# 0xPARC/plonkathon

Measured on NVIDIA H100. Metric: plonk_proofs_per_s_2^20_gates, higher is better.
Workload: dtype u256 (BN254 Fr/Fq integers, 8x32-bit Montgomery limbs)

## Files before the change

plonkathon_b200/csrc/prover.cu:

```cuda
#include <algorithm>
#include <cerrno>
#include <sys/random.h>

#include "common.cuh"
#include "comm.cuh"
#include "transcript.cuh"
#include "prover.cuh"
#include "memory_plan.cuh"

namespace pb200 {

void ntt_run(Context* ctx, const Fr* in, Fr* out, int log_n, bool inverse, uint64_t n_in, const Fr* in_scale,
             const Fr* out_scale);
void ntt_run_on(Context* ctx, cudaStream_t stream, Fr* tmp, const Fr* in, Fr* out, int log_n, bool inverse,
                uint64_t n_in, const Fr* in_scale, const Fr* out_scale, uint64_t in_mul, uint64_t in_add);
void ntt_run_fold(Context* ctx, cudaStream_t stream, Fr* tmp, const Fr* in, Fr* out, int log_n, bool inverse,
                  uint64_t n_in, const Fr* in_scale, const Fr* out_scale, uint64_t in_mul, uint64_t in_add, uint32_t fold);
void ntt_sharded(Context* ctx, const Fr* const* in, Fr* const* out, int count, int log_n, bool inverse);
void ntt_shard_local(Context* ctx, const Fr* const* in, int count, int log_n, bool inverse, uint64_t in_mul,
                     uint64_t in_add, int log_g, int rank, Comm* cm);
void ntt_shard_combine(Context* ctx, const Fr* sub, uint64_t rank_stride, Fr* out, int log_n, bool inverse,
                       uint64_t limit, const Fr* post_scale, uint32_t* nonzero, int log_g, int rank);
uint32_t msm_default_window(uint64_t n, bool fixed_base);

static void coset_extend(Prover* P, cudaStream_t stream, Fr* tmp, const Fr* coeff, Fr* out, const Fr* shift_pow) {
  ntt_run_fold(P->ctx, stream, tmp, coeff, out, P->log_ext, false, P->n, shift_pow, nullptr, 1, 0, P->fold);
}

static void interpolate(Prover* P, const Fr* const* lag, Fr* const* coeff, int count) {
  if (P->world > 1) {
    ntt_sharded(P->ctx, lag, coeff, count, P->log_n, true);
  } else {
    for (int k = 0; k < count; k++) ntt_run(P->ctx, lag[k], coeff[k], P->log_n, true, P->n, nullptr, nullptr);
  }
}

static void launch_coset_ext_async(Prover* P, int first, int count, int done_event) {
  Context* ctx = P->ctx;
  if (!ctx->aux_stream) {
    PB_CUDA(cudaStreamCreateWithFlags(&ctx->aux_stream, cudaStreamNonBlocking));
    for (auto& e : ctx->aux_ev) PB_CUDA(cudaEventCreateWithFlags(&e, cudaEventDisableTiming));
  }
  P->aux_tmp.ensure(P->n_ext * 32);
  PB_CUDA(cudaEventRecord(ctx->aux_ev[3], ctx->stream));
  PB_CUDA(cudaStreamWaitEvent(ctx->aux_stream, ctx->aux_ev[3], 0));
  for (int k = first; k < first + count; k++) {
    coset_extend(P, ctx->aux_stream, P->aux_tmp.as<Fr>(), P->coeff[k].as<Fr>(), P->ext[k].as<Fr>(), P->gpow.as<Fr>());
    if (k == 3 && P->zw_separate)
      coset_extend(P, ctx->aux_stream, P->aux_tmp.as<Fr>(), P->coeff[3].as<Fr>(), P->ext[5].as<Fr>(), P->gpow_w.as<Fr>());
  }
  PB_CUDA(cudaEventRecord(ctx->aux_ev[done_event], ctx->aux_stream));
}
void launch_powers(Context* ctx, Fr* out, uint64_t n, const Fr& base, const Fr& scale);
Fr fr_from_u64(uint64_t x);
Fr fr_root_of_unity(int log_n);
void fr_to_mont(Context* ctx, const Fr* in, Fr* out, uint64_t n);
struct Srs;
void srs_msm(Context* ctx, Srs* srs, const Fr* d_scalars, uint64_t m, bool scalars_mont, uint8_t* out_xy, int* is_identity);
uint64_t srs_size(Srs* s);

#define PB_GRID(n, t) (unsigned)(((n) + (t)-1) / (t)), (t)

__device__ __forceinline__ Fr ldg_fr(const Fr* p) {
  const uint4* q = reinterpret_cast<const uint4*>(p);
  uint4 a = __ldg(q), b = __ldg(q + 1);
  Fr r;
  r.v[0] = a.x; r.v[1] = a.y; r.v[2] = a.z; r.v[3] = a.w;
  r.v[4] = b.x; r.v[5] = b.y; r.v[6] = b.z; r.v[7] = b.w;
  return r;
}

static Fr load_fr_checked(const uint8_t* h) {
  Fr a;
  memcpy(a.v, h, 32);
  PB_CHECK(fp_is_canonical(a), "public input not reduced below the field modulus");
  return a;
}

// ... 198 lines not shown
  if (j < n4) den[j] = fp_mul(n_mont, fp_sub(ldg_fr(X + j), wi));
}

struct QuotientArgs {
  const Fr *A, *B, *C, *Z, *Zw, *PI;
  const Fr *QL, *QR, *QM, *QO, *QC, *S1, *S2, *S3;
  const Fr *L0, *X;
  Fr zh_inv[4];
  Fr alpha, alpha2, beta, gamma, one;
  uint64_t n4;
  uint64_t zw_shift;
  uint32_t world, rank;
  int pi_cnt;
  const Fr* pi_basis[8];
  Fr pi_coef[8];
  CustomTerms custom;
};
struct ZkCoset { Fr w[4][12]; };
struct ZkNextCoset { Fr w[4][24]; };
template <bool ZK_NEXT> struct ZkCosetOf { using type = ZkCoset; };
template <> struct ZkCosetOf<true> { using type = ZkNextCoset; };
static_assert(sizeof(QuotientArgs) + sizeof(Fr*) + sizeof(ZkNextCoset) <= 4096,
              "k_quotient's parameters must fit the 4 KiB parameter space");
template <bool ZK, bool NEXT>
__global__ void __launch_bounds__(128) k_quotient(QuotientArgs q, Fr* T, typename ZkCosetOf<ZK && NEXT>::type zk) {
  uint64_t j = (uint64_t)blockIdx.x * blockDim.x + threadIdx.x;
  if (j >= q.n4) return;
  uint64_t jw = j + q.zw_shift >= q.n4 ? j + q.zw_shift - q.n4 : j + q.zw_shift;
  Fr a = ldg_fr(q.A + j), b = ldg_fr(q.B + j), c = ldg_fr(q.C + j);
  auto quad = [&](Fr y, int i) {
    if constexpr (ZK && NEXT) {
      const uint32_t k = (uint32_t)j & 3;
      const Fr x = ldg_fr(q.X + j);
      y = fp_add(y, fp_add(fp_mul(fp_add(fp_mul(zk.w[k][i], x), zk.w[k][i + 1]), x), zk.w[k][i + 2]));
    }
    return y;
  };
  if constexpr (ZK && NEXT) {
    a = quad(a, 0);
    b = quad(b, 3);
    c = quad(c, 6);
  } else if constexpr (ZK) {
    const uint32_t k = (uint32_t)(j * q.world + q.rank) & 3;
    const Fr x = ldg_fr(q.X + j);
    a = fp_add(a, fp_add(fp_mul(zk.w[k][0], x), zk.w[k][1]));
    b = fp_add(b, fp_add(fp_mul(zk.w[k][2], x), zk.w[k][3]));
    c = fp_add(c, fp_add(fp_mul(zk.w[k][4], x), zk.w[k][5]));
  }
  Fr gate = fp_mul(a, ldg_fr(q.QL + j));
  gate = fp_add(gate, fp_mul(b, ldg_fr(q.QR + j)));
  gate = fp_add(gate, fp_mul(fp_mul(a, b), ldg_fr(q.QM + j)));
  gate = fp_add(gate, fp_mul(c, ldg_fr(q.QO + j)));
  Fr pi = Fr::zero();
  if (q.pi_cnt > 0) {
    for (int i = 0; i < q.pi_cnt; i++) pi = fp_add(pi, fp_mul(q.pi_coef[i], ldg_fr(q.pi_basis[i] + j)));
  } else if (q.PI) {
    pi = ldg_fr(q.PI + j);
  }
  gate = fp_add(gate, fp_add(pi, ldg_fr(q.QC + j)));
  if constexpr (NEXT) {
    const Fr an = quad(ldg_fr(q.A + jw), 15), bn = quad(ldg_fr(q.B + jw), 18), cn = quad(ldg_fr(q.C + jw), 21);
    gate = custom_gate_sum_next(q.custom, j, a, b, c, an, bn, cn, gate);
  } else {
    gate = custom_gate_sum(q.custom, j, a, b, c, gate);
  }
  Fr ag = fp_add(a, q.gamma), bg = fp_add(b, q.gamma), cg = fp_add(c, q.gamma);
  Fr bx = fp_mul(q.beta, ldg_fr(q.X + j));
  Fr bx2 = fp_dbl(bx), bx3 = fp_add(bx2, bx);
  Fr z = ldg_fr(q.Z + j), zw = ldg_fr(q.Zw + jw);
  if constexpr (ZK && NEXT) {
    z = quad(z, 9);
    zw = quad(zw, 12);
  } else if constexpr (ZK) {
    const uint32_t k = (uint32_t)(j * q.world + q.rank) & 3;
    const Fr x = ldg_fr(q.X + j);
    z = fp_add(z, fp_add(fp_mul(fp_add(fp_mul(zk.w[k][6], x), zk.w[k][7]), x), zk.w[k][8]));
    zw = fp_add(zw, fp_add(fp_mul(fp_add(fp_mul(zk.w[k][9], x), zk.w[k][10]), x), zk.w[k][11]));
  }
  Fr p1 = fp_mul(fp_mul(fp_mul(fp_add(ag, bx), fp_add(bg, bx2)), fp_add(cg, bx3)), z);
  Fr p2 = fp_mul(fp_mul(fp_mul(fp_add(ag, fp_mul(q.beta, ldg_fr(q.S1 + j))), fp_add(bg, fp_mul(q.beta, ldg_fr(q.S2 + j)))),
                        fp_add(cg, fp_mul(q.beta, ldg_fr(q.S3 + j)))),
                 zw);
  Fr perm = fp_mul(q.alpha, fp_sub(p1, p2));
  Fr l0 = fp_mul(q.alpha2, fp_mul(fp_sub(z, q.one), ldg_fr(q.L0 + j)));
  Fr num = fp_add(fp_add(gate, perm), l0);
  T[j] = fp_mul(num, q.zh_inv[(j * q.world + q.rank) & 3]);
}

__global__ void k_count_nonzero(const Fr* v, uint64_t n, uint32_t* cnt) {
  uint64_t i = (uint64_t)blockIdx.x * blockDim.x + threadIdx.x;
  if (i < n && !ldg_fr(v + i).is_zero()) atomicAdd(cnt, 1u);
}

struct EvalArgs { const Fr* poly[8]; Fr x_nc[8]; uint64_t n; uint32_t NC; };
__global__ void __launch_bounds__(128) k_horner_strided(EvalArgs a, Fr* H) {
  uint32_t c = blockIdx.x * blockDim.x + threadIdx.x;
  uint32_t p = blockIdx.y;
  if (c >= a.NC) return;
  const Fr* co = a.poly[p];
  uint64_t steps = a.n / a.NC;
  Fr acc = Fr::zero();
  for (uint64_t k = steps; k-- > 0;) acc = fp_add(fp_mul(acc, a.x_nc[p]), ldg_fr(co + k * a.NC + c));
  H[(uint64_t)p * a.NC + c] = acc;
}

struct LinCombArgs { const Fr* vec[26]; Fr w[26]; Fr c0; int count; uint64_t n, first; };
static_assert(5 + PB_MAX_CUSTOM + 10 + 7 <= 26, "round 5's largest batch must fit LinCombArgs");
static_assert(5 + PB_MAX_CUSTOM + 10 + 3 <= 26, "round 5's batch with a shuffle must fit LinCombArgs");
static_assert(7 + 1 <= 26, "round 5's zero-knowledge tail with a shuffle must fit LinCombArgs");
// ... 95 lines not shown

struct LookupChallenges { Fr delta, eps, one_d, eps_one_d; };
__global__ void k_lookup_z2_terms(const Fr* t, const Fr* f, const Fr* h1, const Fr* h2, LookupChallenges ch, uint64_t n,
                                  Fr* num, Fr* den) {
  uint64_t i = (uint64_t)blockIdx.x * blockDim.x + threadIdx.x;
  if (i >= n) return;
  const uint64_t i1 = i + 1 == n ? 0 : i + 1;
  const Fr x1 = ldg_fr(h1 + i), x2 = ldg_fr(h2 + i);
  num[i] = fp_mul(fp_mul(ch.one_d, fp_add(ch.eps, ldg_fr(f + i))),
                  fp_add(fp_add(ch.eps_one_d, ldg_fr(t + i)), fp_mul(ch.delta, ldg_fr(t + i1))));
  den[i] = fp_mul(fp_add(fp_add(ch.eps_one_d, x1), fp_mul(ch.delta, x2)),
                  fp_add(fp_add(ch.eps_one_d, x2), fp_mul(ch.delta, ldg_fr(h1 + i1))));
}

struct LookupQuotientArgs {
  const Fr *A, *B, *C, *QK, *QT, *T, *F, *H1, *H2, *Z2, *L0;
  Fr zh_inv[4];
  Fr eta, eta2, eta3, delta, eps, one_d, eps_one_d, alpha3, alpha4, alpha5, one;
  uint64_t n4;
};
struct ZkLookupCoset { const Fr* X; Fr w[4][18]; };
static_assert(sizeof(LookupQuotientArgs) + sizeof(Fr*) + sizeof(ZkLookupCoset) <= 4096,
              "k_quotient_lookup's parameters must fit the 4 KiB parameter space");
template <bool ZK>
__global__ void __launch_bounds__(128) k_quotient_lookup(LookupQuotientArgs q, Fr* out, ZkLookupCoset zk) {
  uint64_t j = (uint64_t)blockIdx.x * blockDim.x + threadIdx.x;
  if (j >= q.n4) return;
  const uint64_t jw = j + 4 >= q.n4 ? j + 4 - q.n4 : j + 4;
  const uint32_t k = (uint32_t)j & 3;
  const Fr x = ZK ? ldg_fr(zk.X + j) : Fr::zero();
  auto lin = [&](Fr y, int i) {
    if constexpr (ZK) y = fp_add(y, fp_add(fp_mul(zk.w[k][i], x), zk.w[k][i + 1]));
    return y;
  };
  auto quad = [&](Fr y, int i) {
    if constexpr (ZK) y = fp_add(y, fp_add(fp_mul(fp_add(fp_mul(zk.w[k][i], x), zk.w[k][i + 1]), x), zk.w[k][i + 2]));
    return y;
  };
  const Fr f = lin(ldg_fr(q.F + j), 2);
  Fr w = lin(fp_add(ldg_fr(q.A + j), fp_add(fp_mul(q.eta, ldg_fr(q.B + j)), fp_mul(q.eta2, ldg_fr(q.C + j)))), 0);
  Fr acc = fp_mul(ldg_fr(q.QK + j), fp_sub(w, f));
  if (q.QT) acc = fp_add(acc, fp_mul(q.eta3, ldg_fr(q.QT + j)));
  acc = fp_mul(q.alpha3, acc);
  const Fr z2 = quad(ldg_fr(q.Z2 + j), 12), h1 = quad(ldg_fr(q.H1 + j), 4), h2 = lin(ldg_fr(q.H2 + j), 10);
  Fr p1 = fp_mul(fp_mul(fp_mul(z2, q.one_d), fp_add(q.eps, f)),
                 fp_add(fp_add(q.eps_one_d, ldg_fr(q.T + j)), fp_mul(q.delta, ldg_fr(q.T + jw))));
  Fr p2 = fp_mul(fp_mul(quad(ldg_fr(q.Z2 + jw), 15), fp_add(fp_add(q.eps_one_d, h1), fp_mul(q.delta, h2))),
                 fp_add(fp_add(q.eps_one_d, h2), fp_mul(q.delta, quad(ldg_fr(q.H1 + jw), 7))));
  acc = fp_add(acc, fp_mul(q.alpha4, fp_sub(p1, p2)));
  acc = fp_add(acc, fp_mul(q.alpha5, fp_mul(fp_sub(z2, q.one), ldg_fr(q.L0 + j))));
  out[j] = fp_add(out[j], fp_mul(acc, q.zh_inv[j & 3]));
}

struct ShuffleChallenges { Fr theta, theta2, kappa; };
__global__ void k_shuffle_terms(const Fr* A, const Fr* B, const Fr* C, const Fr* QIN, const Fr* QOUT,
                                ShuffleChallenges ch, uint64_t n, Fr* num, Fr* den) {
  uint64_t i = (uint64_t)blockIdx.x * blockDim.x + threadIdx.x;
  if (i >= n) return;
  const Fr t = fp_add(ch.kappa, fp_add(ldg_fr(A + i), fp_add(fp_mul(ch.theta, ldg_fr(B + i)),
                                                              fp_mul(ch.theta2, ldg_fr(C + i)))));
  num[i] = ldg_fr(QIN + i).is_zero() ? Fr::one() : t;
  den[i] = ldg_fr(QOUT + i).is_zero() ? Fr::one() : t;
}

struct ShuffleQuotientArgs {
  const Fr *A, *B, *C, *QIN, *QOUT, *Z3, *L0;
  Fr zh_inv[4];
  Fr theta, theta2, kappa_m1, alpha3, alpha4, one;
  uint64_t n4;
};
struct ZkShuffleCoset { const Fr* X; Fr w[4][9]; };
static_assert(sizeof(ShuffleQuotientArgs) + sizeof(Fr*) + sizeof(ZkShuffleCoset) <= 4096,
              "k_quotient_shuffle's parameters must fit the 4 KiB parameter space");
template <bool ZK>
__global__ void __launch_bounds__(128) k_quotient_shuffle(ShuffleQuotientArgs q, Fr* out, ZkShuffleCoset zk) {
  uint64_t j = (uint64_t)blockIdx.x * blockDim.x + threadIdx.x;
  if (j >= q.n4) return;
  const uint64_t jw = j + 4 >= q.n4 ? j + 4 - q.n4 : j + 4;
  const uint32_t kz = (uint32_t)j & 3;
  const Fr x = ZK ? ldg_fr(zk.X + j) : Fr::zero();
  auto quad = [&](Fr y, int i) {
    if constexpr (ZK) y = fp_add(y, fp_add(fp_mul(fp_add(fp_mul(zk.w[kz][i], x), zk.w[kz][i + 1]), x), zk.w[kz][i + 2]));
    return y;
  };
  const Fr k = fp_add(q.kappa_m1, quad(fp_add(ldg_fr(q.A + j), fp_add(fp_mul(q.theta, ldg_fr(q.B + j)),
                                                                        fp_mul(q.theta2, ldg_fr(q.C + j)))), 0));
  const Fr z3 = quad(ldg_fr(q.Z3 + j), 3);
  Fr acc = fp_sub(fp_mul(quad(ldg_fr(q.Z3 + jw), 6), fp_add(q.one, fp_mul(ldg_fr(q.QOUT + j), k))),
                  fp_mul(z3, fp_add(q.one, fp_mul(ldg_fr(q.QIN + j), k))));
  acc = fp_add(fp_mul(q.alpha3, acc), fp_mul(q.alpha4, fp_mul(fp_sub(z3, q.one), ldg_fr(q.L0 + j))));
  out[j] = fp_add(out[j], fp_mul(acc, q.zh_inv[j & 3]));
}


static void upload_mont(Context* ctx, DevBuf& dst, const uint8_t* h, uint64_t n) {
  dst.ensure(n * 32);
  PB_CUDA(cudaMemcpyAsync(dst.p, h, n * 32, cudaMemcpyHostToDevice, ctx->stream));
  fr_to_mont(ctx, dst.as<Fr>(), dst.as<Fr>(), n);
}

Comm* ctx_comm(Context* ctx);

static void ensure_pi_basis(Prover* P, int count) {
  Context* ctx = P->ctx;
  const uint64_t n = P->n, ne = P->n_ext;
  cudaStream_t st = ctx->stream;
  if ((int)P->pi_basis.size() >= count) return;
  Fr w = fr_root_of_unity(P->log_n);
  DevBuf den(ne * 32);
  for (int i = (int)P->pi_basis.size(); i < count; i++) {
    Fr wi = fp_pow_u64(w, (uint64_t)i);
    Four zh;
    for (int k = 0; k < 4; k++) zh.v[k] = fp_mul(wi, P->zh[k]);
    P->pi_basis.emplace_back(ne * 32);
// ... 120 lines not shown
  for (int k = 0; k < Prover::CUSTOM0 + n_custom; k++) {
    upload_mont(ctx, P->sel_lag[k], k < Prover::CUSTOM0 ? h_pk[k] : h_custom[k - Prover::CUSTOM0], n);
    P->sel_coeff[k].alloc(n * 32);
    ntt_run(ctx, P->sel_lag[k].as<Fr>(), P->sel_coeff[k].as<Fr>(), log_n, true, n, nullptr, nullptr);
    P->sel_ext[k].alloc(ne * 32);
    if (!P->sliced)
      coset_extend(P.get(), st, nullptr, P->sel_coeff[k].as<Fr>(), P->sel_ext[k].as<Fr>(), P->gpow.as<Fr>());
  }
  for (int k = 0; k < 4; k++) P->lag[k].alloc(n * 32);
  for (int k = 0; k < 5; k++) { P->coeff[k].alloc(n * 32); P->ext[k].alloc(ne * 32); }
  if (P->zw_separate) P->ext[5].alloc(ne * 32);
  P->pi_lag.alloc(n * 32);
  if (P->world > 1) {
    P->tq.alloc(3 * n * 32);
    P->tq_loc.alloc(ne * 32);
  } else if (P->sliced) {
    P->tq.alloc(3 * n * 32);
  } else {
    P->tq.alloc(n4 * 32);
  }
  for (int k = 0; k < 5; k++) P->tmp[k].alloc(n * 32);
  P->flags.alloc(64);
  if (const char* e = getenv("PB200_OVERLAP")) P->overlap = atoi(e) != 0;
  if (P->sliced) P->overlap = false;
  PB_CUDA(cudaStreamSynchronize(st));
  PB_CUDA(cudaGetLastError());
  return P.release();
}

void prover_destroy(Prover* p) { delete p; }

static uint32_t read_flag(Prover* P, int idx) {
  uint32_t v;
  PB_CUDA(cudaMemcpyAsync(&v, P->flags.as<uint32_t>() + idx, 4, cudaMemcpyDeviceToHost, P->ctx->stream));
  PB_CUDA(cudaStreamSynchronize(P->ctx->stream));
  return v;
}

Comm* ctx_comm(Context* ctx);

static void eval_polys(Prover* P, int count, const Fr* const* polys, const Fr* xs, Fr* out) {
  Context* ctx = P->ctx;
  const uint64_t n = P->n / (uint64_t)P->world, lo = n * (uint64_t)P->rank;
  uint32_t NC1 = (uint32_t)std::min<uint64_t>(n, 4096);
  uint32_t NC2 = std::min<uint32_t>(NC1, 32);
  ctx->scratch[0].ensure((size_t)count * (NC1 + NC2) * 32);
// ... 604 lines not shown
    slice_lagrange(P, r, 0, Fr::one(), P->pi_basis[0].as<Fr>());
    if (P->pi_sparse) {
      bool first = true;
      for (uint64_t i = 0; i < P->n_public; i++) {
        if (P->pub_neg[i].is_zero()) continue;
        slice_lagrange(P, r, i, P->pub_neg[i], first ? P->ext[4].as<Fr>() : P->tmp[1].as<Fr>());
        if (!first) fr_vec_op(ctx, 0, P->ext[4].as<Fr>(), P->tmp[1].as<Fr>(), Fr::zero(), P->ext[4].as<Fr>(), n, 0);
        first = false;
      }
      if (first && P->n_public) PB_CUDA(cudaMemsetAsync(P->ext[4].p, 0, n * 32, st));
    }
    q.rank = (uint32_t)r;
    Fr* slot = ctx->gather.as<Fr>() + (uint64_t)r * n;
    k_quotient<false, false><<<PB_GRID(n, 128), 0, st>>>(q, slot, zk);
    ctx->launches++;
    const Fr* te = slot;
    ntt_shard_local(ctx, &te, 1, P->log_n + 2, true, 1, 0, 2, r, nullptr);
  }
  PB_CUDA(cudaMemsetAsync(P->flags.p, 0, 64, st));
  ntt_shard_combine(ctx, ctx->gather.as<Fr>(), n, P->tq.as<Fr>(), P->log_n + 2, true, 3 * n, P->ginv_pow.as<Fr>(),
                    P->flags.as<uint32_t>(), 2, 0);
}

void prover_round3(Prover* P, const Fr& alpha_c, const Fr& cofactor_c) {
  Context* ctx = P->ctx;
  const uint64_t n = P->n, n4 = 4 * n, ne = P->n_ext;
  cudaStream_t st = ctx->stream;
  P->alpha = fp_to_mont(alpha_c);
  P->fft_cofactor = fp_to_mont(cofactor_c);
  if (P->sliced) {
    quotient_sliced(P);
    PB_CHECK(read_flag(P, 0) == 0, "AssertionError: quotient has degree >= 3n (prover.py:205-208)");
    const Fr* t123[3] = {P->tq.as<Fr>(), P->tq.as<Fr>() + n, P->tq.as<Fr>() + 2 * n};
    P->commit_batch(t123, 3, n, P->fields[F_T_LO]);
    return;
  }
  if (P->overlap) {
    PB_CUDA(cudaStreamWaitEvent(st, ctx->aux_ev[0], 0));
    PB_CUDA(cudaStreamWaitEvent(st, ctx->aux_ev[1], 0));
  }
  for (int k = (P->overlap ? 4 : 0); k < (P->pi_sparse ? 4 : 5); k++) {
    coset_extend(P, st, nullptr, P->coeff[k].as<Fr>(), P->ext[k].as<Fr>(), P->gpow.as<Fr>());
    if (k == 3 && P->zw_separate)
      coset_extend(P, st, nullptr, P->coeff[3].as<Fr>(), P->ext[5].as<Fr>(), P->gpow_w.as<Fr>());
  }
  QuotientArgs q;
  q.pi_cnt = P->pi_sparse ? (int)P->n_public : 0;
  for (int i = 0; i < q.pi_cnt; i++) { q.pi_basis[i] = P->pi_basis[i].as<Fr>(); q.pi_coef[i] = P->pub_neg[i]; }
  q.A = P->ext[0].as<Fr>(); q.B = P->ext[1].as<Fr>(); q.C = P->ext[2].as<Fr>(); q.Z = P->ext[3].as<Fr>();
  q.Zw = P->zw_separate ? P->ext[5].as<Fr>() : P->ext[3].as<Fr>();
  q.zw_shift = P->zw_shift;
  q.world = (uint32_t)P->world;
  q.rank = (uint32_t)P->rank;
  q.PI = P->pi_sparse ? nullptr : P->ext[4].as<Fr>();
  q.QM = P->sel_ext[Prover::QM].as<Fr>(); q.QL = P->sel_ext[Prover::QL].as<Fr>(); q.QR = P->sel_ext[Prover::QR].as<Fr>();
  q.QO = P->sel_ext[Prover::QO].as<Fr>(); q.QC = P->sel_ext[Prover::QC].as<Fr>();
  q.S1 = P->sel_ext[Prover::S1].as<Fr>(); q.S2 = P->sel_ext[Prover::S2].as<Fr>(); q.S3 = P->sel_ext[Prover::S3].as<Fr>();
  q.custom = P->custom_terms(P->sel_ext);
  q.L0 = P->pi_basis[0].as<Fr>(); q.X = P->xs.as<Fr>();
  for (int k = 0; k < 4; k++) q.zh_inv[k] = P->zh_inv[k];
  q.alpha = P->alpha; q.alpha2 = fp_sqr(P->alpha); q.beta = P->beta; q.gamma = P->gamma; q.one = Fr::one();
  q.n4 = ne;
  Fr* t_evals = P->world > 1 ? P->tq_loc.as<Fr>() : P->tq.as<Fr>();
  ZkCoset zk{};
  if (P->next_row && P->zk) {
    const Fr* b = P->zk_b;
    const Fr w = fr_root_of_unity(P->log_n), w2 = fp_sqr(w);
    const Fr per[24] = {b[11], b[0], b[1], b[12], b[2], b[3], b[13], b[4], b[5], b[6], b[7], b[8],
                        fp_mul(b[6], w2), fp_mul(b[7], w), b[8], fp_mul(b[11], w2), fp_mul(b[0], w), b[1],
                        fp_mul(b[12], w2), fp_mul(b[2], w), b[3], fp_mul(b[13], w2), fp_mul(b[4], w), b[5]};
    ZkNextCoset zn;
    for (int k = 0; k < 4; k++)
      for (int i = 0; i < 24; i++) zn.w[k][i] = fp_mul(per[i], P->zh[k]);
    k_quotient<true, true><<<PB_GRID(ne, 128), 0, st>>>(q, t_evals, zn);
  } else if (P->next_row) {
    k_quotient<false, true><<<PB_GRID(ne, 128), 0, st>>>(q, t_evals, zk);
  } else if (P->zk) {
    const Fr* b = P->zk_b;
    const Fr w = fr_root_of_unity(P->log_n);
    const Fr per[12] = {b[0], b[1], b[2], b[3], b[4], b[5], b[6], b[7], b[8], fp_mul(b[6], fp_sqr(w)), fp_mul(b[7], w), b[8]};
    for (int k = 0; k < 4; k++)
      for (int i = 0; i < 12; i++) zk.w[k][i] = fp_mul(per[i], P->zh[k]);
    k_quotient<true, false><<<PB_GRID(ne, 128), 0, st>>>(q, t_evals, zk);
  } else {
    k_quotient<false, false><<<PB_GRID(ne, 128), 0, st>>>(q, t_evals, zk);
  }
  ctx->launches++;
  if (P->lk) {
    for (int k = 0; k < Prover::LK_VECS; k++)
      coset_extend(P, st, nullptr, P->lk_coeff[k].as<Fr>(), P->lk_ext[k].as<Fr>(), P->gpow.as<Fr>());
    LookupQuotientArgs lq;
    lq.A = q.A; lq.B = q.B; lq.C = q.C; lq.QK = P->lk_qk_ext.as<Fr>(); lq.L0 = q.L0;
    lq.QT = P->lk_tagged ? P->lk_qt_ext.as<Fr>() : nullptr;
    lq.T = P->lk_ext[Prover::LK_T].as<Fr>(); lq.F = P->lk_ext[Prover::LK_F].as<Fr>();
    lq.H1 = P->lk_ext[Prover::LK_H1].as<Fr>(); lq.H2 = P->lk_ext[Prover::LK_H2].as<Fr>();
    lq.Z2 = P->lk_ext[Prover::LK_Z2].as<Fr>();
    for (int k = 0; k < 4; k++) lq.zh_inv[k] = P->zh_inv[k];
    lq.eta = P->eta; lq.eta2 = fp_sqr(P->eta); lq.eta3 = fp_mul(lq.eta2, P->eta); lq.delta = P->delta; lq.eps = P->epsilon;
    lq.one_d = fp_add(Fr::one(), P->delta); lq.eps_one_d = fp_mul(P->epsilon, lq.one_d);
    lq.alpha3 = fp_mul(q.alpha2, P->alpha); lq.alpha4 = fp_sqr(q.alpha2); lq.alpha5 = fp_mul(lq.alpha4, P->alpha);
    lq.one = Fr::one();
    lq.n4 = ne;
    ZkLookupCoset zl{};
    if (P->zk) {
      const Fr* b = P->zk_b;
      const Fr w = fr_root_of_unity(P->log_n), w2 = fp_sqr(w);
      const Fr e1 = fp_add(b[0], fp_add(fp_mul(lq.eta, b[2]), fp_mul(lq.eta2, b[4])));
      const Fr e0 = fp_add(b[1], fp_add(fp_mul(lq.eta, b[3]), fp_mul(lq.eta2, b[5])));
      const Fr per[18] = {e1,    e0,    b[11], b[12], b[13], b[14], b[15], fp_mul(b[13], w2), fp_mul(b[14], w),
                          b[15], b[16], b[17], b[18], b[19], b[20], fp_mul(b[18], w2), fp_mul(b[19], w), b[20]};
      zl.X = P->xs.as<Fr>();
      for (int k = 0; k < 4; k++)
        for (int i = 0; i < 18; i++) zl.w[k][i] = fp_mul(per[i], P->zh[k]);
      k_quotient_lookup<true><<<PB_GRID(ne, 128), 0, st>>>(lq, t_evals, zl);
    } else {
      k_quotient_lookup<false><<<PB_GRID(ne, 128), 0, st>>>(lq, t_evals, zl);
    }
    ctx->launches++;
  }
  if (P->sh) {
    coset_extend(P, st, nullptr, P->sh_z3_coeff.as<Fr>(), P->sh_z3_ext.as<Fr>(), P->gpow.as<Fr>());
    ShuffleQuotientArgs sq;
    sq.A = q.A; sq.B = q.B; sq.C = q.C; sq.L0 = q.L0;
    sq.QIN = P->sh_ext[Prover::SH_IN].as<Fr>(); sq.QOUT = P->sh_ext[Prover::SH_OUT].as<Fr>();
    sq.Z3 = P->sh_z3_ext.as<Fr>();
    for (int k = 0; k < 4; k++) sq.zh_inv[k] = P->zh_inv[k];
    sq.theta = P->theta; sq.theta2 = fp_sqr(P->theta); sq.kappa_m1 = fp_sub(P->kappa, Fr::one());
    sq.alpha3 = fp_mul(q.alpha2, P->alpha); sq.alpha4 = fp_sqr(q.alpha2); sq.one = Fr::one();
    sq.n4 = ne;
    ZkShuffleCoset zs{};
    if (P->zk) {
      const Fr *b = P->zk_b, *c = P->zk_z3_b();
      const Fr w = fr_root_of_unity(P->log_n), w2 = fp_sqr(w);
      auto wsum = [&](const Fr& x, const Fr& y, const Fr& z) {
        return fp_add(x, fp_add(fp_mul(sq.theta, y), fp_mul(sq.theta2, z)));
      };
      const Fr e2 = P->next_row ? wsum(b[11], b[12], b[13]) : Fr::zero();
      const Fr per[9] = {e2,   wsum(b[0], b[2], b[4]), wsum(b[1], b[3], b[5]), c[0], c[1], c[2],
                         fp_mul(c[0], w2), fp_mul(c[1], w), c[2]};
      zs.X = P->xs.as<Fr>();
      for (int k = 0; k < 4; k++)
        for (int i = 0; i < 9; i++) zs.w[k][i] = fp_mul(per[i], P->zh[k]);
      k_quotient_shuffle<true><<<PB_GRID(ne, 128), 0, st>>>(sq, t_evals, zs);
    } else {
      k_quotient_shuffle<false><<<PB_GRID(ne, 128), 0, st>>>(sq, t_evals, zs);
    }
    ctx->launches++;
  }
  PB_CUDA(cudaMemsetAsync(P->flags.p, 0, 64, st));
  if (P->world > 1) {
    const Fr* te = t_evals;
    ntt_shard_local(ctx, &te, 1, P->log_n + 2, true, 1, 0, P->log_world, P->rank, ctx_comm(ctx));
    ntt_shard_combine(ctx, ctx->gather.as<Fr>(), ne, P->tq.as<Fr>(), P->log_n + 2, true, 3 * n,
                      P->ginv_pow.as<Fr>(), P->flags.as<uint32_t>(), P->log_world, P->rank);
  } else {
    ntt_run(ctx, P->tq.as<Fr>(), P->tq.as<Fr>(), P->log_n + 2, true, n4, nullptr, P->ginv_pow.as<Fr>());
    const uint64_t top = P->zk ? P->zk_t3_len() + 2 * n : 3 * n;
    k_count_nonzero<<<PB_GRID(n4 - top, 256), 0, st>>>(P->tq.as<Fr>() + top, n4 - top, P->flags.as<uint32_t>());
    ctx->launches++;
  }
  if (P->zk) {
    PB_CHECK(read_flag(P, 0) == 0, P->next_row
                 ? "AssertionError: quotient has degree >= 3n + 9 (zero-knowledge mode, next-row terms; prover.py:205-208)"
                 : "AssertionError: quotient has degree >= 3n + 6 (zero-knowledge mode; prover.py:205-208)");
    const Fr* t = P->tq.as<Fr>();
    const Fr b10 = P->zk_b[9], b11 = P->zk_b[10], zero = Fr::zero();
    zk_blind(P, t, n, ZkPatch{{zero, zero, zero}, {b10, zero, zero}}, P->zk_t[0].as<Fr>());
    zk_blind(P, t + n, n, ZkPatch{{fp_neg(b10), zero, zero}, {b11, zero, zero}}, P->zk_t[1].as<Fr>());
    const uint64_t t3 = P->zk_t3_len();
    zk_blind(P, t + 2 * n, t3, ZkPatch{{fp_neg(b11), zero, zero}, {zero, zero, zero}}, P->zk_t[2].as<Fr>());
// ... 318 lines not shown
```

plonkathon_b200/csrc/prover.cuh:

```cuda
#pragma once
#include "common.cuh"
#include "proof_layout.cuh"

namespace pb200 {

struct Srs;
void srs_msm(Context* ctx, Srs* srs, const Fr* d_scalars, uint64_t m, bool scalars_mont, uint8_t* out_xy, int* is_identity);
void srs_msm_batch(Context* ctx, Srs* srs, const Fr* const* d_scalars, uint32_t batch, uint64_t m, bool scalars_mont,
                   uint8_t* out_xy, int* is_identity);
void srs_msm_batch_partial(Context* ctx, Srs* srs, const Fr* const* d_scalars, uint32_t batch, uint64_t first,
                           uint64_t count, uint32_t bucket_lo, uint32_t bucket_hi, bool scalars_mont, G1XYZZ* out);
void srs_msm_batch_sharded(Context* ctx, Srs* srs, const Fr* const* d_scalars, uint32_t batch, uint64_t m,
                           bool scalars_mont, uint8_t* out_xy, int* is_identity);
uint32_t srs_bucket_count(Srs* s);

#define PB_MAX_CUSTOM 4
#define PB_SLICED_WHY "not available on a sliced prover (its 4n-coset cache does not fit in device memory, or PB200_SLICED=1): "
#define PB_FACTOR_ONE 6
struct CustomTerms {
  const Fr* Q[PB_MAX_CUSTOM];
  uint8_t f[PB_MAX_CUSTOM][3];
  int count;
};
PB_HD Fr custom_monomial(const Fr& a, const Fr& b, const Fr& c, const uint8_t* f) {
// ... 46 lines not shown
PB_HD int lookup_cmp(const Fr* x, const Fr (&y)[4], int width) {
#pragma unroll
  for (int w = 0; w < 4; w++) {
    if (w == width) break;
#pragma unroll
    for (int l = 7; l >= 0; l--)
      if (x[w].v[l] != y[w].v[l]) return x[w].v[l] < y[w].v[l] ? -1 : 1;
  }
  return 0;
}

struct Prover {
  Context* ctx;
  Srs* srs;
  int log_n;
  uint64_t n;
  int world = 1, rank = 0, log_world = 0;
  int log_ext = 0;
  uint64_t n_ext = 0;
  uint32_t fold = 1;
  uint64_t zw_shift = 4;
  bool zw_separate = false;
  bool sliced = false;
  DevBuf sel_coeff[8 + PB_MAX_CUSTOM];
  DevBuf sel_lag[8 + PB_MAX_CUSTOM];
  DevBuf sel_ext[8 + PB_MAX_CUSTOM];
  int n_custom = 0;
  uint8_t custom_f[PB_MAX_CUSTOM][3];
  bool next_row = false;
  Fr nr_ev[3];
  DevBuf roots;
  DevBuf gpow;
  DevBuf gpow_w;
  DevBuf ginv_pow;
  DevBuf xs;
  Fr g, g_inv, zh_inv[4];
  Fr zh[4];
  DevBuf lag[4];
  DevBuf coeff[5];
  DevBuf pi_lag;
  DevBuf ext[6];
  DevBuf tq;
  DevBuf tq_loc;
  DevBuf tmp[5];
  DevBuf aux_tmp;
  bool overlap = true;
// ... 87 lines not shown
```

Before: 24.63.

## Evaluate quotient on three size-n coset slices instead of the 4n coset

Round 3 now evaluates the quotient numerator on three shifted size-n cosets (three of the four sub-cosets of the 4n extended domain) instead of the full 4n extension. Each slice is inverse-transformed and combined with precomputed Lagrange-style weights to recover the three degree-n quotient chunks. The intent is to remove a quarter of the extension NTTs and quotient-kernel work plus the final large inverse NTT. Correctness relies on the quotient having degree below 3n, so a one-point check on the fourth sub-coset is added, which costs extra polynomial evaluations and a host sync. The path is limited to the single-device, non-ZK case.

```diff
diff --git a/plonkathon_b200/csrc/prover.cu b/plonkathon_b200/csrc/prover.cu
--- a/plonkathon_b200/csrc/prover.cu
+++ b/plonkathon_b200/csrc/prover.cu
@@ -1,5 +1,6 @@
 #include <algorithm>
 #include <cerrno>
+#include <cstring>
 #include <sys/random.h>
 
 #include "common.cuh"
@@ -22,9 +23,31 @@
 void ntt_shard_combine(Context* ctx, const Fr* sub, uint64_t rank_stride, Fr* out, int log_n, bool inverse,
                        uint64_t limit, const Fr* post_scale, uint32_t* nonzero, int log_g, int rank);
 uint32_t msm_default_window(uint64_t n, bool fixed_base);
+void launch_powers(Context* ctx, Fr* out, uint64_t n, const Fr& base, const Fr& scale);
+Fr fr_from_u64(uint64_t x);
+Fr fr_root_of_unity(int log_n);
 
 static void coset_extend(Prover* P, cudaStream_t stream, Fr* tmp, const Fr* coeff, Fr* out, const Fr* shift_pow) {
   ntt_run_fold(P->ctx, stream, tmp, coeff, out, P->log_ext, false, P->n, shift_pow, nullptr, 1, 0, P->fold);
+}
+
+static const Fr* slice_shift(Prover* P, int r) {
+  return r == 0 ? P->gpow.as<Fr>() : P->aux_tmp.as<Fr>() + (uint64_t)r * P->n;
+}
+static void slice_shifts(Prover* P) {
+  P->aux_tmp.ensure(P->n_ext * 32);
+  const Fr mu = fr_root_of_unity(P->log_n + 2);
+  for (int r = 1; r < 3; r++)
+    launch_powers(P->ctx, P->aux_tmp.as<Fr>() + (uint64_t)r * P->n, P->n, fp_mul(P->g, fp_pow_u64(mu, r)), Fr::one());
+}
+static void extend(Prover* P, cudaStream_t stream, Fr* tmp, const Fr* coeff, Fr* out) {
+  if (!P->three_slices()) {
+    coset_extend(P, stream, tmp, coeff, out, P->gpow.as<Fr>());
+    return;
+  }
+  for (int r = 0; r < 3; r++)
+    ntt_run_fold(P->ctx, stream, tmp, coeff, out + (uint64_t)r * P->n, P->log_n, false, P->n, slice_shift(P, r), nullptr,
+                 1, 0, 1);
 }
 
 static void interpolate(Prover* P, const Fr* const* lag, Fr* const* coeff, int count) {
@@ -42,18 +65,18 @@
     for (auto& e : ctx->aux_ev) PB_CUDA(cudaEventCreateWithFlags(&e, cudaEventDisableTiming));
   }
   P->aux_tmp.ensure(P->n_ext * 32);
+  const bool three = P->three_slices();
+  if (first == 0 && three) slice_shifts(P);
+  get_plan(ctx, three ? P->log_n : P->log_ext, false);
   PB_CUDA(cudaEventRecord(ctx->aux_ev[3], ctx->stream));
   PB_CUDA(cudaStreamWaitEvent(ctx->aux_stream, ctx->aux_ev[3], 0));
   for (int k = first; k < first + count; k++) {
-    coset_extend(P, ctx->aux_stream, P->aux_tmp.as<Fr>(), P->coeff[k].as<Fr>(), P->ext[k].as<Fr>(), P->gpow.as<Fr>());
+    extend(P, ctx->aux_stream, P->aux_tmp.as<Fr>(), P->coeff[k].as<Fr>(), P->ext[k].as<Fr>());
     if (k == 3 && P->zw_separate)
       coset_extend(P, ctx->aux_stream, P->aux_tmp.as<Fr>(), P->coeff[3].as<Fr>(), P->ext[5].as<Fr>(), P->gpow_w.as<Fr>());
   }
   PB_CUDA(cudaEventRecord(ctx->aux_ev[done_event], ctx->aux_stream));
 }
-void launch_powers(Context* ctx, Fr* out, uint64_t n, const Fr& base, const Fr& scale);
-Fr fr_from_u64(uint64_t x);
-Fr fr_root_of_unity(int log_n);
 void fr_to_mont(Context* ctx, const Fr* in, Fr* out, uint64_t n);
 struct Srs;
 void srs_msm(Context* ctx, Srs* srs, const Fr* d_scalars, uint64_t m, bool scalars_mont, uint8_t* out_xy, int* is_identity);
@@ -298,11 +321,21 @@
 template <> struct ZkCosetOf<true> { using type = ZkNextCoset; };
 static_assert(sizeof(QuotientArgs) + sizeof(Fr*) + sizeof(ZkNextCoset) <= 4096,
               "k_quotient's parameters must fit the 4 KiB parameter space");
-template <bool ZK, bool NEXT>
+__device__ __forceinline__ void slice_point(uint64_t t, uint64_t n, uint64_t& s, uint64_t& w, uint32_t& r) {
+  r = (uint32_t)(t >= n) + (uint32_t)(t >= 2 * n);
+  const uint64_t j = t - r * n;
+  s = 4 * j + r;
+  w = j + 1 == n ? t + 1 - n : t + 1;
+}
+template <bool ZK, bool NEXT, bool SLICES = false>
 __global__ void __launch_bounds__(128) k_quotient(QuotientArgs q, Fr* T, typename ZkCosetOf<ZK && NEXT>::type zk) {
+  static_assert(!(ZK && SLICES), "zero knowledge keeps the 4n coset");
   uint64_t j = (uint64_t)blockIdx.x * blockDim.x + threadIdx.x;
   if (j >= q.n4) return;
   uint64_t jw = j + q.zw_shift >= q.n4 ? j + q.zw_shift - q.n4 : j + q.zw_shift;
+  uint64_t s = j;
+  uint32_t r = 0;
+  if constexpr (SLICES) slice_point(j, q.n4 / 3, s, jw, r);
   Fr a = ldg_fr(q.A + j), b = ldg_fr(q.B + j), c = ldg_fr(q.C + j);
   auto quad = [&](Fr y, int i) {
     if constexpr (ZK && NEXT) {
@@ -323,25 +356,25 @@
     b = fp_add(b, fp_add(fp_mul(zk.w[k][2], x), zk.w[k][3]));
     c = fp_add(c, fp_add(fp_mul(zk.w[k][4], x), zk.w[k][5]));
   }
-  Fr gate = fp_mul(a, ldg_fr(q.QL + j));
-  gate = fp_add(gate, fp_mul(b, ldg_fr(q.QR + j)));
-  gate = fp_add(gate, fp_mul(fp_mul(a, b), ldg_fr(q.QM + j)));
-  gate = fp_add(gate, fp_mul(c, ldg_fr(q.QO + j)));
+  Fr gate = fp_mul(a, ldg_fr(q.QL + s));
+  gate = fp_add(gate, fp_mul(b, ldg_fr(q.QR + s)));
+  gate = fp_add(gate, fp_mul(fp_mul(a, b), ldg_fr(q.QM + s)));
+  gate = fp_add(gate, fp_mul(c, ldg_fr(q.QO + s)));
   Fr pi = Fr::zero();
   if (q.pi_cnt > 0) {
-    for (int i = 0; i < q.pi_cnt; i++) pi = fp_add(pi, fp_mul(q.pi_coef[i], ldg_fr(q.pi_basis[i] + j)));
+    for (int i = 0; i < q.pi_cnt; i++) pi = fp_add(pi, fp_mul(q.pi_coef[i], ldg_fr(q.pi_basis[i] + s)));
   } else if (q.PI) {
     pi = ldg_fr(q.PI + j);
   }
-  gate = fp_add(gate, fp_add(pi, ldg_fr(q.QC + j)));
+  gate = fp_add(gate, fp_add(pi, ldg_fr(q.QC + s)));
   if constexpr (NEXT) {
     const Fr an = quad(ldg_fr(q.A + jw), 15), bn = quad(ldg_fr(q.B + jw), 18), cn = quad(ldg_fr(q.C + jw), 21);
-    gate = custom_gate_sum_next(q.custom, j, a, b, c, an, bn, cn, gate);
+    gate = custom_gate_sum_next(q.custom, s, a, b, c, an, bn, cn, gate);
   } else {
-    gate = custom_gate_sum(q.custom, j, a, b, c, gate);
+    gate = custom_gate_sum(q.custom, s, a, b, c, gate);
   }
   Fr ag = fp_add(a, q.gamma), bg = fp_add(b, q.gamma), cg = fp_add(c, q.gamma);
-  Fr bx = fp_mul(q.beta, ldg_fr(q.X + j));
+  Fr bx = fp_mul(q.beta, ldg_fr(q.X + s));
   Fr bx2 = fp_dbl(bx), bx3 = fp_add(bx2, bx);
   Fr z = ldg_fr(q.Z + j), zw = ldg_fr(q.Zw + jw);
   if constexpr (ZK && NEXT) {
@@ -354,13 +387,26 @@
     zw = fp_add(zw, fp_add(fp_mul(fp_add(fp_mul(zk.w[k][9], x), zk.w[k][10]), x), zk.w[k][11]));
   }
   Fr p1 = fp_mul(fp_mul(fp_mul(fp_add(ag, bx), fp_add(bg, bx2)), fp_add(cg, bx3)), z);
-  Fr p2 = fp_mul(fp_mul(fp_mul(fp_add(ag, fp_mul(q.beta, ldg_fr(q.S1 + j))), fp_add(bg, fp_mul(q.beta, ldg_fr(q.S2 + j)))),
-                        fp_add(cg, fp_mul(q.beta, ldg_fr(q.S3 + j)))),
+  Fr p2 = fp_mul(fp_mul(fp_mul(fp_add(ag, fp_mul(q.beta, ldg_fr(q.S1 + s))), fp_add(bg, fp_mul(q.beta, ldg_fr(q.S2 + s)))),
+                        fp_add(cg, fp_mul(q.beta, ldg_fr(q.S3 + s)))),
                  zw);
   Fr perm = fp_mul(q.alpha, fp_sub(p1, p2));
-  Fr l0 = fp_mul(q.alpha2, fp_mul(fp_sub(z, q.one), ldg_fr(q.L0 + j)));
+  Fr l0 = fp_mul(q.alpha2, fp_mul(fp_sub(z, q.one), ldg_fr(q.L0 + s)));
   Fr num = fp_add(fp_add(gate, perm), l0);
-  T[j] = fp_mul(num, q.zh_inv[(j * q.world + q.rank) & 3]);
+  T[j] = fp_mul(num, q.zh_inv[SLICES ? r : (j * q.world + q.rank) & 3]);
+}
+
+struct SliceCombine { Fr w[3][3]; };
+__global__ void __launch_bounds__(128) k_slices_combine(Fr* T, const Fr* X, const Fr* ginv_pow, uint64_t n,
+                                                        SliceCombine m) {
+  uint64_t i = (uint64_t)blockIdx.x * blockDim.x + threadIdx.x;
+  if (i >= n) return;
+  const Fr x = ldg_fr(X + (i == 0 ? 0 : 4 * n - i));
+  const Fr e0 = T[i], e1 = fp_mul(T[n + i], x), e2 = fp_mul(T[2 * n + i], fp_sqr(x));
+  const Fr gi = ldg_fr(ginv_pow + i);
+#pragma unroll
+  for (int k = 0; k < 3; k++)
+    T[k * n + i] = fp_mul(gi, fp_add(fp_add(fp_mul(m.w[k][0], e0), fp_mul(m.w[k][1], e1)), fp_mul(m.w[k][2], e2)));
 }
 
 __global__ void k_count_nonzero(const Fr* v, uint64_t n, uint32_t* cnt) {
@@ -502,11 +548,15 @@
 struct ZkLookupCoset { const Fr* X; Fr w[4][18]; };
 static_assert(sizeof(LookupQuotientArgs) + sizeof(Fr*) + sizeof(ZkLookupCoset) <= 4096,
               "k_quotient_lookup's parameters must fit the 4 KiB parameter space");
-template <bool ZK>
+template <bool ZK, bool SLICES = false>
 __global__ void __launch_bounds__(128) k_quotient_lookup(LookupQuotientArgs q, Fr* out, ZkLookupCoset zk) {
+  static_assert(!(ZK && SLICES), "zero knowledge keeps the 4n coset");
   uint64_t j = (uint64_t)blockIdx.x * blockDim.x + threadIdx.x;
   if (j >= q.n4) return;
-  const uint64_t jw = j + 4 >= q.n4 ? j + 4 - q.n4 : j + 4;
+  uint64_t jw = j + 4 >= q.n4 ? j + 4 - q.n4 : j + 4;
+  uint64_t s = j;
+  uint32_t r = 0;
+  if constexpr (SLICES) slice_point(j, q.n4 / 3, s, jw, r);
   const uint32_t k = (uint32_t)j & 3;
   const Fr x = ZK ? ldg_fr(zk.X + j) : Fr::zero();
   auto lin = [&](Fr y, int i) {
@@ -519,8 +569,8 @@
   };
   const Fr f = lin(ldg_fr(q.F + j), 2);
   Fr w = lin(fp_add(ldg_fr(q.A + j), fp_add(fp_mul(q.eta, ldg_fr(q.B + j)), fp_mul(q.eta2, ldg_fr(q.C + j)))), 0);
-  Fr acc = fp_mul(ldg_fr(q.QK + j), fp_sub(w, f));
-  if (q.QT) acc = fp_add(acc, fp_mul(q.eta3, ldg_fr(q.QT + j)));
+  Fr acc = fp_mul(ldg_fr(q.QK + s), fp_sub(w, f));
+  if (q.QT) acc = fp_add(acc, fp_mul(q.eta3, ldg_fr(q.QT + s)));
   acc = fp_mul(q.alpha3, acc);
   const Fr z2 = quad(ldg_fr(q.Z2 + j), 12), h1 = quad(ldg_fr(q.H1 + j), 4), h2 = lin(ldg_fr(q.H2 + j), 10);
   Fr p1 = fp_mul(fp_mul(fp_mul(z2, q.one_d), fp_add(q.eps, f)),
@@ -528,8 +578,8 @@
   Fr p2 = fp_mul(fp_mul(quad(ldg_fr(q.Z2 + jw), 15), fp_add(fp_add(q.eps_one_d, h1), fp_mul(q.delta, h2))),
                  fp_add(fp_add(q.eps_one_d, h2), fp_mul(q.delta, quad(ldg_fr(q.H1 + jw), 7))));
   acc = fp_add(acc, fp_mul(q.alpha4, fp_sub(p1, p2)));
-  acc = fp_add(acc, fp_mul(q.alpha5, fp_mul(fp_sub(z2, q.one), ldg_fr(q.L0 + j))));
-  out[j] = fp_add(out[j], fp_mul(acc, q.zh_inv[j & 3]));
+  acc = fp_add(acc, fp_mul(q.alpha5, fp_mul(fp_sub(z2, q.one), ldg_fr(q.L0 + s))));
+  out[j] = fp_add(out[j], fp_mul(acc, q.zh_inv[SLICES ? r : j & 3]));
 }
 
 struct ShuffleChallenges { Fr theta, theta2, kappa; };
@@ -552,11 +602,15 @@
 struct ZkShuffleCoset { const Fr* X; Fr w[4][9]; };
 static_assert(sizeof(ShuffleQuotientArgs) + sizeof(Fr*) + sizeof(ZkShuffleCoset) <= 4096,
               "k_quotient_shuffle's parameters must fit the 4 KiB parameter space");
-template <bool ZK>
+template <bool ZK, bool SLICES = false>
 __global__ void __launch_bounds__(128) k_quotient_shuffle(ShuffleQuotientArgs q, Fr* out, ZkShuffleCoset zk) {
+  static_assert(!(ZK && SLICES), "zero knowledge keeps the 4n coset");
   uint64_t j = (uint64_t)blockIdx.x * blockDim.x + threadIdx.x;
   if (j >= q.n4) return;
-  const uint64_t jw = j + 4 >= q.n4 ? j + 4 - q.n4 : j + 4;
+  uint64_t jw = j + 4 >= q.n4 ? j + 4 - q.n4 : j + 4;
+  uint64_t s = j;
+  uint32_t r = 0;
+  if constexpr (SLICES) slice_point(j, q.n4 / 3, s, jw, r);
   const uint32_t kz = (uint32_t)j & 3;
   const Fr x = ZK ? ldg_fr(zk.X + j) : Fr::zero();
   auto quad = [&](Fr y, int i) {
@@ -566,10 +620,10 @@
   const Fr k = fp_add(q.kappa_m1, quad(fp_add(ldg_fr(q.A + j), fp_add(fp_mul(q.theta, ldg_fr(q.B + j)),
                                                                         fp_mul(q.theta2, ldg_fr(q.C + j)))), 0));
   const Fr z3 = quad(ldg_fr(q.Z3 + j), 3);
-  Fr acc = fp_sub(fp_mul(quad(ldg_fr(q.Z3 + jw), 6), fp_add(q.one, fp_mul(ldg_fr(q.QOUT + j), k))),
-                  fp_mul(z3, fp_add(q.one, fp_mul(ldg_fr(q.QIN + j), k))));
-  acc = fp_add(fp_mul(q.alpha3, acc), fp_mul(q.alpha4, fp_mul(fp_sub(z3, q.one), ldg_fr(q.L0 + j))));
-  out[j] = fp_add(out[j], fp_mul(acc, q.zh_inv[j & 3]));
+  Fr acc = fp_sub(fp_mul(quad(ldg_fr(q.Z3 + jw), 6), fp_add(q.one, fp_mul(ldg_fr(q.QOUT + s), k))),
+                  fp_mul(z3, fp_add(q.one, fp_mul(ldg_fr(q.QIN + s), k))));
+  acc = fp_add(fp_mul(q.alpha3, acc), fp_mul(q.alpha4, fp_mul(fp_sub(z3, q.one), ldg_fr(q.L0 + s))));
+  out[j] = fp_add(out[j], fp_mul(acc, q.zh_inv[SLICES ? r : j & 3]));
 }
 
 
@@ -736,6 +790,7 @@
   for (int k = 0; k < 5; k++) P->tmp[k].alloc(n * 32);
   P->flags.alloc(64);
   if (const char* e = getenv("PB200_OVERLAP")) P->overlap = atoi(e) != 0;
+  if (const char* e = getenv("PB200_ROUND3")) P->round3_slices = strcmp(e, "4n") != 0;
   if (P->sliced) P->overlap = false;
   PB_CUDA(cudaStreamSynchronize(st));
   PB_CUDA(cudaGetLastError());
@@ -1386,6 +1441,102 @@
                     P->flags.as<uint32_t>(), 2, 0);
 }
 
+static SliceCombine slice_combine_weights(const Prover* P) {
+  Fr X[3];
+  for (int r = 0; r < 3; r++) X[r] = fp_add(P->zh[r], Fr::one());
+  SliceCombine m;
+  Fr g_r = Fr::one();
+  for (int r = 0; r < 3; r++) {
+    const Fr &xs = X[(r + 1) % 3], &xt = X[(r + 2) % 3];
+    const Fr d = fp_mul(g_r, fp_inv(fp_mul(fp_sub(X[r], xs), fp_sub(X[r], xt))));
+    m.w[0][r] = fp_mul(fp_mul(xs, xt), d);
+    m.w[1][r] = fp_neg(fp_mul(fp_add(xs, xt), d));
+    m.w[2][r] = d;
+    g_r = fp_mul(g_r, P->g_inv);
+  }
+  return m;
+}
+
+static bool quotient_matches_on_slice3(Prover* P, QuotientArgs q, const LookupQuotientArgs* lk,
+                                       const ShuffleQuotientArgs* sh) {
+  Context* ctx = P->ctx;
+  const uint64_t n = P->n;
+  cudaStream_t st = ctx->stream;
+  const Fr x = fp_mul(P->g, fp_pow_u64(fr_root_of_unity(P->log_n + 2), 3)), xw = fp_mul(x, fr_root_of_unity(P->log_n));
+  std::vector<const Fr*> polys;
+  std::vector<Fr> at;
+  std::vector<int> slot;
+  int vecs = 0;
+  auto add = [&](const Fr* p, bool next) {
+    polys.push_back(p); at.push_back(x); slot.push_back(5 * vecs);
+    if (next) { polys.push_back(p); at.push_back(xw); slot.push_back(5 * vecs + 4); }
+    return vecs++;
+  };
+  const int vA = add(P->coeff[0].as<Fr>(), P->next_row), vB = add(P->coeff[1].as<Fr>(), P->next_row);
+  const int vC = add(P->coeff[2].as<Fr>(), P->next_row), vZ = add(P->coeff[3].as<Fr>(), true);
+  const int vPI = q.PI ? add(P->coeff[4].as<Fr>(), false) : -1;
+  int vLK = -1, vZ3 = -1;
+  if (lk) {
+    vLK = add(P->lk_coeff[Prover::LK_T].as<Fr>(), true);
+    add(P->lk_coeff[Prover::LK_F].as<Fr>(), false);
+    add(P->lk_coeff[Prover::LK_H1].as<Fr>(), true);
+    add(P->lk_coeff[Prover::LK_H2].as<Fr>(), false);
+    add(P->lk_coeff[Prover::LK_Z2].as<Fr>(), true);
+  }
+  if (sh) vZ3 = add(P->sh_z3_coeff.as<Fr>(), true);
+  for (int k = 0; k < 3; k++) { polys.push_back(P->tq.as<Fr>() + (uint64_t)k * n); at.push_back(x); slot.push_back(-1); }
+  std::vector<Fr> val(polys.size());
+  for (size_t e = 0; e < polys.size(); e += 8)
+    eval_polys(P, (int)std::min<size_t>(8, polys.size() - e), polys.data() + e, at.data() + e, val.data() + e);
+  std::vector<Fr> h((size_t)5 * vecs + 5, Fr::zero());
+  for (size_t e = 0; e < polys.size(); e++)
+    if (slot[e] >= 0) h[slot[e]] = val[e];
+  const size_t E = polys.size();
+  const Fr xn = fp_add(P->zh[3], Fr::one());
+  const Fr t_at = fp_add(val[E - 3], fp_mul(xn, fp_add(val[E - 2], fp_mul(xn, val[E - 1]))));
+  ctx->scratch[0].ensure(h.size() * 32);
+  Fr* d = ctx->scratch[0].as<Fr>();
+  PB_CUDA(cudaMemcpyAsync(d, h.data(), h.size() * 32, cudaMemcpyHostToDevice, st));
+  Fr* out = d + (size_t)5 * vecs;
+  auto v = [&](int i) { return d + (size_t)5 * i; };
+  q.A = v(vA); q.B = v(vB); q.C = v(vC); q.Z = q.Zw = v(vZ);
+  q.PI = vPI >= 0 ? v(vPI) : nullptr;
+  q.zw_shift = 4; q.world = 1; q.rank = 0; q.n4 = 5;
+  q.zh_inv[0] = P->zh_inv[3];
+  for (const Fr** c : {&q.QM, &q.QL, &q.QR, &q.QO, &q.QC, &q.S1, &q.S2, &q.S3, &q.L0, &q.X}) *c += 3;
+  for (int i = 0; i < q.pi_cnt; i++) q.pi_basis[i] += 3;
+  for (int k = 0; k < q.custom.count; k++) q.custom.Q[k] += 3;
+  const ZkCoset zk{};
+  if (P->next_row) k_quotient<false, true><<<1, 128, 0, st>>>(q, out, zk);
+  else k_quotient<false, false><<<1, 128, 0, st>>>(q, out, zk);
+  ctx->launches++;
+  if (lk) {
+    LookupQuotientArgs l = *lk;
+    l.A = q.A; l.B = q.B; l.C = q.C; l.L0 = q.L0;
+    l.QK += 3;
+    if (l.QT) l.QT += 3;
+    l.T = v(vLK); l.F = v(vLK + 1); l.H1 = v(vLK + 2); l.H2 = v(vLK + 3); l.Z2 = v(vLK + 4);
+    l.zh_inv[0] = P->zh_inv[3];
+    l.n4 = 5;
+    k_quotient_lookup<false><<<1, 128, 0, st>>>(l, out, ZkLookupCoset{});
+    ctx->launches++;
+  }
+  if (sh) {
+    ShuffleQuotientArgs s = *sh;
+    s.A = q.A; s.B = q.B; s.C = q.C; s.L0 = q.L0;
+    s.QIN += 3; s.QOUT += 3;
+    s.Z3 = v(vZ3);
+    s.zh_inv[0] = P->zh_inv[3];
+    s.n4 = 5;
+    k_quotient_shuffle<false><<<1, 128, 0, st>>>(s, out, ZkShuffleCoset{});
+    ctx->launches++;
+  }
+  Fr num;
+  PB_CUDA(cudaMemcpyAsync(&num, out, 32, cudaMemcpyDeviceToHost, st));
+  PB_CUDA(cudaStreamSynchronize(st));
+  return fp_sub(num, t_at).is_zero();
+}
+
 void prover_round3(Prover* P, const Fr& alpha_c, const Fr& cofactor_c) {
   Context* ctx = P->ctx;
   const uint64_t n = P->n, n4 = 4 * n, ne = P->n_ext;
@@ -1399,12 +1550,15 @@
     P->commit_batch(t123, 3, n, P->fields[F_T_LO]);
     return;
   }
+  const bool three = P->three_slices();
   if (P->overlap) {
     PB_CUDA(cudaStreamWaitEvent(st, ctx->aux_ev[0], 0));
     PB_CUDA(cudaStreamWaitEvent(st, ctx->aux_ev[1], 0));
+  } else if (three) {
+    slice_shifts(P);
   }
   for (int k = (P->overlap ? 4 : 0); k < (P->pi_sparse ? 4 : 5); k++) {
-    coset_extend(P, st, nullptr, P->coeff[k].as<Fr>(), P->ext[k].as<Fr>(), P->gpow.as<Fr>());
+    extend(P, st, nullptr, P->coeff[k].as<Fr>(), P->ext[k].as<Fr>());
     if (k == 3 && P->zw_separate)
       coset_extend(P, st, nullptr, P->coeff[3].as<Fr>(), P->ext[5].as<Fr>(), P->gpow_w.as<Fr>());
   }
@@ -1424,10 +1578,13 @@
   q.L0 = P->pi_basis[0].as<Fr>(); q.X = P->xs.as<Fr>();
   for (int k = 0; k < 4; k++) q.zh_inv[k] = P->zh_inv[k];
   q.alpha = P->alpha; q.alpha2 = fp_sqr(P->alpha); q.beta = P->beta; q.gamma = P->gamma; q.one = Fr::one();
-  q.n4 = ne;
+  q.n4 = three ? 3 * n : ne;
   Fr* t_evals = P->world > 1 ? P->tq_loc.as<Fr>() : P->tq.as<Fr>();
   ZkCoset zk{};
-  if (P->next_row && P->zk) {
+  if (three) {
+    if (P->next_row) k_quotient<false, true, true><<<PB_GRID(3 * n, 128), 0, st>>>(q, t_evals, zk);
+    else k_quotient<false, false, true><<<PB_GRID(3 * n, 128), 0, st>>>(q, t_evals, zk);
+  } else if (P->next_row && P->zk) {
     const Fr* b = P->zk_b;
     const Fr w = fr_root_of_unity(P->log_n), w2 = fp_sqr(w);
     const Fr per[24] = {b[11], b[0], b[1], b[12], b[2], b[3], b[13], b[4], b[5], b[6], b[7], b[8],
@@ -1450,10 +1607,11 @@
     k_quotient<false, false><<<PB_GRID(ne, 128), 0, st>>>(q, t_evals, zk);
   }
   ctx->launches++;
+  LookupQuotientArgs lq;
+  ShuffleQuotientArgs sq;
   if (P->lk) {
     for (int k = 0; k < Prover::LK_VECS; k++)
-      coset_extend(P, st, nullptr, P->lk_coeff[k].as<Fr>(), P->lk_ext[k].as<Fr>(), P->gpow.as<Fr>());
-    LookupQuotientArgs lq;
+      extend(P, st, nullptr, P->lk_coeff[k].as<Fr>(), P->lk_ext[k].as<Fr>());
     lq.A = q.A; lq.B = q.B; lq.C = q.C; lq.QK = P->lk_qk_ext.as<Fr>(); lq.L0 = q.L0;
     lq.QT = P->lk_tagged ? P->lk_qt_ext.as<Fr>() : nullptr;
     lq.T = P->lk_ext[Prover::LK_T].as<Fr>(); lq.F = P->lk_ext[Prover::LK_F].as<Fr>();
@@ -1464,9 +1622,11 @@
     lq.one_d = fp_add(Fr::one(), P->delta); lq.eps_one_d = fp_mul(P->epsilon, lq.one_d);
     lq.alpha3 = fp_mul(q.alpha2, P->alpha); lq.alpha4 = fp_sqr(q.alpha2); lq.alpha5 = fp_mul(lq.alpha4, P->alpha);
     lq.one = Fr::one();
-    lq.n4 = ne;
+    lq.n4 = three ? 3 * n : ne;
     ZkLookupCoset zl{};
-    if (P->zk) {
+    if (three) {
+      k_quotient_lookup<false, true><<<PB_GRID(3 * n, 128), 0, st>>>(lq, t_evals, zl);
+    } else if (P->zk) {
       const Fr* b = P->zk_b;
       const Fr w = fr_root_of_unity(P->log_n), w2 = fp_sqr(w);
       const Fr e1 = fp_add(b[0], fp_add(fp_mul(lq.eta, b[2]), fp_mul(lq.eta2, b[4])));
@@ -1483,17 +1643,18 @@
     ctx->launches++;
   }
   if (P->sh) {
-    coset_extend(P, st, nullptr, P->sh_z3_coeff.as<Fr>(), P->sh_z3_ext.as<Fr>(), P->gpow.as<Fr>());
-    ShuffleQuotientArgs sq;
+    extend(P, st, nullptr, P->sh_z3_coeff.as<Fr>(), P->sh_z3_ext.as<Fr>());
     sq.A = q.A; sq.B = q.B; sq.C = q.C; sq.L0 = q.L0;
     sq.QIN = P->sh_ext[Prover::SH_IN].as<Fr>(); sq.QOUT = P->sh_ext[Prover::SH_OUT].as<Fr>();
     sq.Z3 = P->sh_z3_ext.as<Fr>();
     for (int k = 0; k < 4; k++) sq.zh_inv[k] = P->zh_inv[k];
     sq.theta = P->theta; sq.theta2 = fp_sqr(P->theta); sq.kappa_m1 = fp_sub(P->kappa, Fr::one());
     sq.alpha3 = fp_mul(q.alpha2, P->alpha); sq.alpha4 = fp_sqr(q.alpha2); sq.one = Fr::one();
-    sq.n4 = ne;
+    sq.n4 = three ? 3 * n : ne;
     ZkShuffleCoset zs{};
-    if (P->zk) {
+    if (three) {
+      k_quotient_shuffle<false, true><<<PB_GRID(3 * n, 128), 0, st>>>(sq, t_evals, zs);
+    } else if (P->zk) {
       const Fr *b = P->zk_b, *c = P->zk_z3_b();
       const Fr w = fr_root_of_unity(P->log_n), w2 = fp_sqr(w);
       auto wsum = [&](const Fr& x, const Fr& y, const Fr& z) {
@@ -1510,6 +1671,20 @@
       k_quotient_shuffle<false><<<PB_GRID(ne, 128), 0, st>>>(sq, t_evals, zs);
     }
     ctx->launches++;
+  }
+  if (three) {
+    for (int r = 0; r < 3; r++) {
+      Fr* d = P->tq.as<Fr>() + (uint64_t)r * n;
+      ntt_run(ctx, d, d, P->log_n, true, n, nullptr, nullptr);
+    }
+    k_slices_combine<<<PB_GRID(n, 128), 0, st>>>(P->tq.as<Fr>(), P->xs.as<Fr>(), P->ginv_pow.as<Fr>(), n,
+                                                   slice_combine_weights(P));
+    ctx->launches++;
+    PB_CHECK(quotient_matches_on_slice3(P, q, P->lk ? &lq : nullptr, P->sh ? &sq : nullptr),
+             "AssertionError: quotient has degree >= 3n (prover.py:205-208)");
+    const Fr* t123[3] = {P->tq.as<Fr>(), P->tq.as<Fr>() + n, P->tq.as<Fr>() + 2 * n};
+    P->commit_batch(t123, 3, n, P->fields[F_T_LO]);
+    return;
   }
   PB_CUDA(cudaMemsetAsync(P->flags.p, 0, 64, st));
   if (P->world > 1) {
diff --git a/plonkathon_b200/csrc/prover.cuh b/plonkathon_b200/csrc/prover.cuh
--- a/plonkathon_b200/csrc/prover.cuh
+++ b/plonkathon_b200/csrc/prover.cuh
@@ -92,6 +92,8 @@
   uint64_t zw_shift = 4;
   bool zw_separate = false;
   bool sliced = false;
+  bool round3_slices = true;
+  bool three_slices() const { return round3_slices && world == 1 && !sliced && !zk; }
   DevBuf sel_coeff[8 + PB_MAX_CUSTOM];
   DevBuf sel_lag[8 + PB_MAX_CUSTOM];
   DevBuf sel_ext[8 + PB_MAX_CUSTOM];
```

After: 25.56, median of 6. 3.8% higher.
